# gio54321/quill-zkvm

Hardware: AMD Instinct MI355X
Metric: G1 MSM scalars/sec at 2^24 + sumcheck-prover ms at 2^20 vars (1/8 GPU) (higher is better)
Workload: dtype u256-montgomery (BN254 Fr scalars, Fq coordinates); 1 GPU; KZG commit / Pippenger G1 MSM, 2^24 BN254 scalars per GPU; parallelism=msm-shard-by-base-index x1

## Files before the change

quill-zkvm_amd/csrc/msm.hip:

```cpp
#include <stdlib.h>
#include <string.h>

#include "common.h"
#include "curve29.h"
#include "msm_plan.h"

using namespace qg;

namespace qg {

static constexpr int MSM_BLOCK = 256;

static int msm_window_bits(size_t n) {
  int best = 4;
  double best_cost = 1e300;
  for (int c = 4; c <= 22; c++) {
    const int W = (255 + c - 1) / c;
    const int k = 254 - c * (W - 1);
    if (k < 30 && (n >> k) > 4096) continue;
    const double cost = (double)n * W + 12.0 * (double)((size_t)1 << (c - 1));
    if (cost < best_cost) {
      best_cost = cost;
      best = c;
    }
// ... 86 lines not shown
    Fr s;
    if (canon_ready) {
      s = canon[i];
    } else {
      s = fr_canon29(scalars[i]);
      canon[i] = s;
    }
    for_each_digit(s, c, W, [&](int w, uint32_t b, bool) {
      if (wsel < 0 || w == wsel) atomicAdd(&hist[b >> LO], 1u);
    });
  }
  __syncthreads();
  for (int g = threadIdx.x; g < H; g += blockDim.x) hrow[(size_t)tb * H + g] = hist[g];
}

__global__ void __launch_bounds__(256)
    k_transpose32(const uint32_t* __restrict__ in, uint32_t rows, uint32_t cols,
                  uint32_t* __restrict__ out) {
  __shared__ uint32_t tile[32][33];
  const uint32_t c0 = blockIdx.x * 32, r0 = blockIdx.y * 32;
  const uint32_t tx = threadIdx.x & 31, ty = threadIdx.x >> 5;
  for (uint32_t k = ty; k < 32; k += 8)
    if (r0 + k < rows && c0 + tx < cols) tile[k][tx] = in[(size_t)(r0 + k) * cols + c0 + tx];
  __syncthreads();
  for (uint32_t k = ty; k < 32; k += 8)
    if (c0 + k < cols && r0 + tx < rows) out[(size_t)(c0 + k) * rows + r0 + tx] = tile[tx][k];
}

template <int BLK>
__device__ void lds_exscan(uint32_t* a, int n, uint32_t* tmp ) {
  const int per = (n + BLK - 1) / BLK;
  const int b = threadIdx.x * per;
  const int lane = threadIdx.x & 63, wid = threadIdx.x >> 6;
  uint32_t tot = 0;
  for (int k = 0; k < per; k++)
    if (b + k < n) tot += a[b + k];
  uint32_t inc = tot;
#pragma unroll
  for (int d = 1; d < 64; d <<= 1) {
    const uint32_t y = __shfl_up(inc, d, 64);
    if (lane >= d) inc += y;
// ... 149 lines not shown
      const uint32_t dst = gb[b >> LO] + p;
      tmp_e[dst] = ent[p];
      tmp_l[dst] = (uint16_t)(b & lmask);
    }
    if (!more) break;
    __syncthreads();
    k = kn;
    if (PF) {
#pragma unroll
      for (int j = 0; j < PER; j++) sv[j] = nsv[j];
      loff = nloff;
    }
  }
}

template <int BLK>
__global__ void __launch_bounds__(BLK)
    k_sortA_rows(uint32_t* __restrict__ hrow, uint32_t* __restrict__ orow, int H) {
  __shared__ uint32_t a[SORT_H_MAX], scr[BLK / 64];
  const size_t r = (size_t)blockIdx.x * H;
  for (int g = threadIdx.x; g < H; g += blockDim.x) a[g] = hrow[r + g];
  __syncthreads();
  lds_exscan<BLK>(a, H, scr);
  for (int g = threadIdx.x; g < H; g += blockDim.x) {
    hrow[r + g] = a[g];
    orow[r + g] -= a[g];
  }
}

__global__ void __launch_bounds__(1024)
    k_sort_chunks(const uint32_t* __restrict__ goff, uint32_t nblk, int H, uint32_t chunk,
                  uint32_t* __restrict__ gstart, uint32_t* __restrict__ cbase,
                  uint32_t* __restrict__ chunk_group, uint32_t* __restrict__ misc) {
  __shared__ uint32_t sh[1024];
  const int g = threadIdx.x;
  if (threadIdx.x >= 1 && threadIdx.x <= 3) misc[threadIdx.x] = threadIdx.x == 2 ? 0xffffffffu : 0u;
  const uint32_t total = goff[(size_t)H * nblk];
  uint32_t gs = 0, ge = 0, nch = 0;
  if (g < H) {
    gs = goff[(size_t)g * nblk];
    ge = (g + 1 < H) ? goff[(size_t)(g + 1) * nblk] : total;
    nch = (ge - gs + chunk - 1) / chunk;
    gstart[g] = gs;
  }
  sh[threadIdx.x] = nch;
  __syncthreads();
  for (int off = 1; off < 1024; off <<= 1) {
    uint32_t add = threadIdx.x >= (unsigned)off ? sh[threadIdx.x - off] : 0u;
    __syncthreads();
    sh[threadIdx.x] += add;
    __syncthreads();
  }
  const uint32_t cb = sh[threadIdx.x] - nch;
  if (g < H) {
    cbase[g] = cb;
    for (uint32_t k = 0; k < nch; k++) chunk_group[cb + k] = (uint32_t)g;
  }
  if (threadIdx.x == 1023) {
    gstart[H] = total;
    cbase[H] = sh[1023];
    misc[0] = sh[1023];
  }
}

template <int BLK, int CHUNK>
__global__ void __launch_bounds__(BLK)
    k_sortB_hist(const uint16_t* __restrict__ tmp_l, const uint32_t* __restrict__ gstart,
                 const uint32_t* __restrict__ cbase, const uint32_t* __restrict__ chunk_group,
                 const uint32_t* __restrict__ nchunks, int NL, uint32_t* __restrict__ chist) {
  extern __shared__ uint32_t hist[];
  const uint32_t nch = *nchunks;
  if (blockIdx.x >= nch) return;
  const uint32_t k = xcd_tile(blockIdx.x, nch);
  const uint32_t g = chunk_group[k];
  const uint32_t s = gstart[g] + (k - cbase[g]) * CHUNK;
  const uint32_t e = min(s + CHUNK, gstart[g + 1]);
// ... 15 lines not shown

__global__ void k_sort_bucket_count(const uint32_t* __restrict__ cbase, const uint32_t* __restrict__ chist,
                                    int LO, uint32_t nb, uint32_t* __restrict__ counts) {
  const uint32_t b = blockIdx.x * blockDim.x + threadIdx.x;
  if (b >= nb) return;
  const uint32_t g = b >> LO, l = b & ((1u << LO) - 1);
  uint32_t c = 0;
#pragma unroll 8
  for (uint32_t k = cbase[g]; k < cbase[g + 1]; k++) c += chist[((size_t)k << LO) + l];
  counts[b] = c;
}

__global__ void k_sort_chunk_offsets(const uint32_t* __restrict__ cbase,
                                     const uint32_t* __restrict__ chist, int LO, uint32_t nb,
                                     const uint32_t* __restrict__ bstart,
                                     uint32_t* __restrict__ coff) {
  const uint32_t b = blockIdx.x * blockDim.x + threadIdx.x;
  if (b >= nb) return;
  const uint32_t g = b >> LO, l = b & ((1u << LO) - 1);
  uint32_t run = bstart[b];
#pragma unroll 8
  for (uint32_t k = cbase[g]; k < cbase[g + 1]; k++) {
    const size_t idx = ((size_t)k << LO) + l;
    coff[idx] = run;
    run += chist[idx];
  }
}

template <int BLK, int CHUNK, bool PF>
__global__ void __launch_bounds__(BLK)
    k_sortB_scatter(const uint32_t* __restrict__ tmp_e, const uint16_t* __restrict__ tmp_l,
                    const uint32_t* __restrict__ gstart,
// ... 124 lines not shown
    if (PF) {
#pragma unroll
      for (int j = 0; j < PER; j++) {
        ev[j] = nev[j];
        lv[j] = nlv[j];
      }
#pragma unroll
      for (int r = 0; r < RPT; r++) co[r] = nco[r];
      loff = nloff;
      s = ns, e = ne;
      nck = fck, ns = fs, ne = fe;
    }
  }
}

__global__ void k_scan32_tiles(const uint32_t* __restrict__ in, size_t n, uint32_t* __restrict__ out,
                               uint32_t* __restrict__ tile_tot) {
  __shared__ uint32_t sh[256];
  const size_t base = ((size_t)blockIdx.x * 256 + threadIdx.x) * 8;
  uint32_t v[8], tot = 0;
  for (int k = 0; k < 8; k++) {
    v[k] = base + k < n ? in[base + k] : 0u;
    tot += v[k];
  }
  sh[threadIdx.x] = tot;
  __syncthreads();
  for (int off = 1; off < 256; off <<= 1) {
    uint32_t add = threadIdx.x >= (unsigned)off ? sh[threadIdx.x - off] : 0u;
    __syncthreads();
    sh[threadIdx.x] += add;
    __syncthreads();
  }
  uint32_t run = sh[threadIdx.x] - tot;
  for (int k = 0; k < 8; k++) {
    if (base + k < n) out[base + k] = run;
    run += v[k];
  }
  if (threadIdx.x == 255) tile_tot[blockIdx.x] = sh[255];
}

__global__ void __launch_bounds__(1024)
    k_scan32_top(uint32_t* __restrict__ tile_tot, int ntiles, uint32_t* __restrict__ out_total) {
  __shared__ uint32_t sh[1024];
  const int per = (ntiles + 1023) / 1024;
  const int base = threadIdx.x * per;
  uint32_t tot = 0;
  for (int k = 0; k < per; k++)
    if (base + k < ntiles) tot += tile_tot[base + k];
  sh[threadIdx.x] = tot;
  __syncthreads();
  for (int off = 1; off < 1024; off <<= 1) {
    uint32_t add = threadIdx.x >= (unsigned)off ? sh[threadIdx.x - off] : 0u;
    __syncthreads();
    sh[threadIdx.x] += add;
    __syncthreads();
  }
  uint32_t run = sh[threadIdx.x] - tot;
  for (int k = 0; k < per; k++) {
    if (base + k < ntiles) {
      uint32_t t = tile_tot[base + k];
      tile_tot[base + k] = run;
      run += t;
    }
  }
  if (threadIdx.x == 1023) *out_total = sh[1023];
}

__global__ void k_scan32_add(const uint32_t* __restrict__ tile_off, size_t n, uint32_t* __restrict__ out) {
  const size_t i = (size_t)blockIdx.x * blockDim.x + threadIdx.x;
  if (i < n) out[i] += tile_off[i / 2048];
}

__device__ __forceinline__ uint2 scan_val(const uint32_t* counts, size_t i, size_t nb, uint32_t L) {
  uint32_t c = i < nb ? counts[i] : 0u;
  return make_uint2(c, (c + L - 1) / L);
}

__global__ void k_scan_tiles(const uint32_t* __restrict__ counts, size_t nb, uint32_t L,
                             uint32_t* __restrict__ bstart, uint2* __restrict__ tile_tot,
                             uint32_t* __restrict__ max_tpb) {
  __shared__ uint2 sh[SCAN_BLOCK];
  size_t base = (size_t)blockIdx.x * SCAN_TILE + threadIdx.x * SCAN_PER_THREAD;
  uint2 v[SCAN_PER_THREAD];
  uint2 tot = make_uint2(0, 0);
  uint32_t mx = 0;
  for (int k = 0; k < SCAN_PER_THREAD; k++) {
    v[k] = scan_val(counts, base + k, nb, L);
    tot.x += v[k].x;
    tot.y += v[k].y;
    mx = max(mx, v[k].y);
  }
  if (mx > 1) atomicMax(max_tpb, mx);
  sh[threadIdx.x] = tot;
  __syncthreads();
  for (int off = 1; off < SCAN_BLOCK; off <<= 1) {
    uint2 add = threadIdx.x >= (unsigned)off ? sh[threadIdx.x - off] : make_uint2(0, 0);
    __syncthreads();
    sh[threadIdx.x].x += add.x;
    sh[threadIdx.x].y += add.y;
    __syncthreads();
  }
  uint2 run = threadIdx.x ? sh[threadIdx.x - 1] : make_uint2(0, 0);
  for (int k = 0; k < SCAN_PER_THREAD; k++) {
    size_t i = base + k;
    if (i < nb) bstart[i] = run.x;
    run.x += v[k].x;
    run.y += v[k].y;
// ... 453 lines not shown
    A_out[w] = x29_store(wsum);
    Y_out[w] = x29_store(Yw);
  }
#endif
}

QG_DEV G1Xyzz x29_export_xyzz(const X29& p) {
  if (x29_is_inf(p)) return G1Xyzz::infinity();
  return {q29_export(p.X), q29_export(p.Y), q29_export(p.ZZ), q29_export(p.ZZZ)};
}

template <bool Q4>
__global__ void __launch_bounds__(64)
    k_msm_wfold(const G1Xyzz* __restrict__ A_in, const G1Xyzz* __restrict__ Y_in, uint32_t m,
                size_t istride, G1Xyzz* __restrict__ A_out, G1Xyzz* __restrict__ Y_out,
                size_t ostride) {
#if defined(__HIP_DEVICE_COMPILE__)
  constexpr uint32_t ES = Q4 ? 4 : 1, G = 64 / ES;
  const uint32_t e0 = blockIdx.x * G, e = e0 + threadIdx.x / ES;
  const uint32_t mv = m - e0 < G ? m - e0 : G;
  X29 A = x29_inf(), Y = x29_inf();
  if (e < m) {
    A = x29_load(A_in[(size_t)blockIdx.y * istride + e]);
    Y = x29_load(Y_in[(size_t)blockIdx.y * istride + e]);
  }
  const int gl = Q4 ? 4 : 6;
  X29 Yw;
  msm_fold<Q4>(A, Y, gl, mv, 0, Y_out ? gl : 0, Yw);
  if (threadIdx.x == 0) {
    const size_t w = (size_t)blockIdx.y * ostride + blockIdx.x;
    if (Y_out) {
      A_out[w] = x29_store(A);
      Y_out[w] = x29_store(Yw);
    } else {
      A_out[w] = x29_export_xyzz(A);
    }
  }
#endif
}

__global__ void k_srs_pack(const G1Affine* __restrict__ pts, size_t n, MsmPt* __restrict__ out) {
  const size_t i = (size_t)blockIdx.x * blockDim.x + threadIdx.x;
  if (i >= n) return;
  const G1Affine w = pts[i];
  out[i] = w.is_inf() ? msm_pt_pack(Q29::zero(), Q29::zero(), true)
                      : msm_pt_pack(q29_import(w.x), q29_import(w.y), false);
}

__global__ void k_srs_unpack(const MsmPt* __restrict__ rows, size_t n, G1Affine* __restrict__ out) {
  const size_t i = (size_t)blockIdx.x * blockDim.x + threadIdx.x;
// ... 113 lines not shown
void srs_unpack_rows(qg_ctx* ctx, const qg_srs* srs, size_t offset, size_t n, G1Affine* d_out) {
  hipLaunchKernelGGL(k_srs_unpack, dim3(div_up(n, 256)), dim3(256), 0, ctx->stream,
                     srs->d_table + offset, n, d_out);
  QG_LAUNCH_CHECK();
}

struct MsmRun {
  bool empty = true;
  uint32_t L = 1, T = 4;
  size_t nslots = 0;
  X29Raw* partial = nullptr;
  uint32_t* owner = nullptr;
  uint32_t* bstart = nullptr;
  uint32_t* misc = nullptr;
  uint32_t* h_mx = nullptr;
  hipEvent_t ev_mx = nullptr;
  uint32_t gen = 0;
};
static constexpr int MSM_MAX_BATCH = 1024;

struct MsmJob {
  const Fr* d_scalars = nullptr;
  size_t n = 0;
  int slot = 0;
  size_t srs_off = 0;
  hipStream_t stream = nullptr;
  uint32_t* hv = nullptr;
  uint32_t hgen = 0;
  int wsel = -1;
  bool canon_ready = false;
// ... 24 lines not shown
  QG_HIP(hipFuncSetAttribute(f.fn, hipFuncAttributeMaxDynamicSharedMemorySize, 160 * 1024));
  ctx->memo[key] = "1";
}

static int sort_pf_occupancy(qg_ctx* ctx, char pass, int blk, size_t smem) {
  QG_CHECK(blk == 1024, QG_ERR_ASSERT, "the prefetching scatters have 1024 threads");
  const SortFn f = pass == 'A' ? sortA_fn<1024, true>() : sortB_fn<1024, 16384, true>();
  sort_lds_attr(ctx, f);
  const std::string mk = f.key + "_occ" + std::to_string(smem);
  auto it = ctx->memo.find(mk);
  if (it != ctx->memo.end()) return std::stoi(it->second);
  int occ = 0;
  QG_HIP(hipOccupancyMaxActiveBlocksPerMultiprocessor(&occ, f.fn, blk, smem));
  ctx->memo[mk] = std::to_string(occ);
  return occ;
}

static MsmPlan msm_job_plan(qg_ctx* ctx, const qg_srs* srs, const MsmJob& job) {
  const int W = srs->W, wsel = job.wsel;
  QG_CHECK((wsel < 0) == (srs->tables == W) && wsel < W, QG_ERR_INVALID,
           "MSM window selection does not match the SRS tables");
  QG_CHECK((size_t)W * srs->n < 0x80000000ull, QG_ERR_UNSUPPORTED, "SRS table index overflow");
  QG_CHECK(job.slot >= 0 && job.slot < MSM_MAX_BATCH, QG_ERR_UNSUPPORTED, "MSM batch too large");
  MsmShape sh;
  sh.n = job.n;
  sh.c = srs->c;
  sh.W = W;
  sh.wsel = wsel;
  sh.side = msm_on_side_stream(ctx, job);
  sh.cus = ctx->num_cus();
  return msm_plan(sh, msm_tuning_from_env(), [ctx](char pass, int blk, size_t smem) {
    return sort_pf_occupancy(ctx, pass, blk, smem);
  });
}

struct MsmScratch {
  uint32_t *ghist, *goff, *gtiles, *gstart, *cbase, *cgroup;
  uint32_t* misc;
  uint32_t *chist, *coff, *tmp_e;
  uint16_t* tmp_l;
  uint32_t *hrow, *orow;
  Fr* canon;
  uint32_t *counts, *bstart, *entries;
  uint2* tile_tot;
  X29Raw* partial;
  uint32_t* owner;
};

static MsmScratch msm_scratch(qg_ctx* ctx, const MsmPlan& p, size_t n, int slot, bool side,
                              bool run) {
  const std::string sfx = "#" + std::to_string(slot);
  const std::string tg = side ? "@" + std::to_string(slot & 1) : std::string();
  constexpr bool RESERVED = true, RUN_ONLY = false;
  auto get = [&](auto*& ptr, const std::string& name, size_t count, bool reserved) {
    using T = std::remove_reference_t<decltype(*ptr)>;
    if (run || reserved) ptr = ctx->scratch_as<T>(name, count);
  };
  MsmScratch s{};
  get(s.ghist, "msm_ghist" + tg, p.nghist + 1, RESERVED);
  get(s.goff, "msm_goff" + tg, p.nghist + 1, RESERVED);
  get(s.gtiles, "msm_gtiles" + tg, div_up(p.nghist, 2048) + 1, RESERVED);
  get(s.gstart, "msm_gstart" + tg, p.H + 1, RESERVED);
  get(s.cbase, "msm_cbase" + tg, p.H + 1, RESERVED);
  get(s.cgroup, "msm_cgroup" + tg, p.max_chunks, RESERVED);
  get(s.misc, "msm_misc" + sfx, 5, RESERVED);
  get(s.chist, "msm_chist" + tg, p.max_chunks * p.NL, RESERVED);
  get(s.coff, "msm_coff" + tg, p.max_chunks * p.NL, RESERVED);
  get(s.tmp_e, "msm_tmp_e" + tg, p.max_entries + 1, RESERVED);
  get(s.tmp_l, "msm_tmp_l" + tg, p.max_entries + 1, RESERVED);
  get(s.hrow, "msm_hrow" + tg, p.nghist + 1, RESERVED);
  get(s.orow, "msm_orow" + tg, p.nghist + 1, RESERVED);
  get(s.canon, "msm_canon" + tg, n, RESERVED);
  get(s.counts, "msm_counts" + tg, p.nb, RESERVED);
  get(s.bstart, "msm_bstart" + sfx, p.nb + 1, RESERVED);
  get(s.entries, "msm_entries" + tg, p.max_entries + 1, RESERVED);
  get(s.tile_tot, "msm_tiles" + tg, p.ntiles, RUN_ONLY);
  get(s.partial, "msm_partial" + sfx, p.nslots, RUN_ONLY);
  get(s.owner, "msm_owner" + sfx, p.nslots, RUN_ONLY);
  return s;
}
// ... 9 lines not shown
}

template <int BLK, bool PF>
static void launch_sortA_scatter(qg_ctx* ctx, const qg_srs* srs, const MsmJob& job,
                                 const MsmPlan& p, const MsmScratch& s) {
  sort_lds_attr(ctx, sortA_fn<BLK, PF>());
  hipLaunchKernelGGL(HIP_KERNEL_NAME(k_sortA_scatter<BLK, PF>), dim3(p.gridA), dim3(BLK), p.smemA,
                     job.stream, s.canon, job.n, srs->n, job.srs_off, srs->c, srs->W, p.LO, p.H,
                     p.nblk, p.geo.tile, s.hrow, s.orow, s.tmp_e, s.tmp_l, job.wsel,
                     PF ? 3u * (uint32_t)p.H : 0u);
  QG_LAUNCH_CHECK();
}
template <int BLK>
static void launch_sortA(qg_ctx* ctx, const qg_srs* srs, const MsmJob& job, const MsmPlan& p,
                         const MsmScratch& s) {
  hipLaunchKernelGGL(k_sortA_rows<BLK>, dim3(p.nblk), dim3(BLK), 0, job.stream, s.hrow, s.orow, p.H);
  QG_LAUNCH_CHECK();
  if (p.pfA)
    launch_sortA_scatter<1024, true>(ctx, srs, job, p, s);
  else
    launch_sortA_scatter<BLK, false>(ctx, srs, job, p, s);
}

template <int BLK, int CHUNK>
static void launch_sortB_hist(const MsmJob& job, const MsmPlan& p, const MsmScratch& s) {
  hipLaunchKernelGGL(HIP_KERNEL_NAME(k_sortB_hist<BLK, CHUNK>), dim3((unsigned)p.max_chunks),
                     dim3(BLK), p.NL * sizeof(uint32_t), job.stream, s.tmp_l, s.gstart, s.cbase,
                     s.cgroup, s.misc, p.NL, s.chist);
  QG_LAUNCH_CHECK();
}
template <int BLK, int CHUNK, bool PF>
static void launch_sortB_scatter_as(qg_ctx* ctx, const MsmJob& job, const MsmPlan& p,
// ... 29 lines not shown
  const bool small = p.geo.chunk == 8192;
  switch (p.geo.blkB) {
    case 256: launch_sortB_scatter<256, 8192>(ctx, job, p, s); break;
    case 512:
      if (small) launch_sortB_scatter<512, 8192>(ctx, job, p, s);
      else launch_sortB_scatter<512, 16384>(ctx, job, p, s);
      break;
    default: launch_sortB_scatter<1024, 16384>(ctx, job, p, s); break;
  }
}

static void msm_passA_launch(qg_ctx* ctx, const qg_srs* srs, const MsmJob& job, const MsmPlan& p,
                             const MsmScratch& s) {
  const hipStream_t st = job.stream;
  const uint32_t nblk = p.nblk, H = (uint32_t)p.H;
  hipLaunchKernelGGL(k_sortA_hist, dim3(nblk), dim3(SORT_BLOCK), H * sizeof(uint32_t), st,
                     job.d_scalars, job.n, srs->c, srs->W, p.LO, p.H, nblk, p.geo.tile, s.hrow,
                     s.canon, job.hv, job.hgen, job.wsel, job.canon_ready ? 1 : 0);
  QG_LAUNCH_CHECK();
  hipLaunchKernelGGL(k_transpose32, dim3(div_up(H, 32), div_up(nblk, 32)), dim3(256), 0, st, s.hrow,
                     nblk, H, s.ghist);
  QG_LAUNCH_CHECK();
  const unsigned gt = div_up(p.nghist, 2048);
  hipLaunchKernelGGL(k_scan32_tiles, dim3(gt), dim3(256), 0, st, s.ghist, p.nghist, s.goff, s.gtiles);
  QG_LAUNCH_CHECK();
  hipLaunchKernelGGL(k_scan32_top, dim3(1), dim3(1024), 0, st, s.gtiles, (int)gt, s.goff + p.nghist);
  QG_LAUNCH_CHECK();
  hipLaunchKernelGGL(k_scan32_add, dim3(div_up(p.nghist, 256)), dim3(256), 0, st, s.gtiles, p.nghist,
                     s.goff);
  QG_LAUNCH_CHECK();
  hipLaunchKernelGGL(k_transpose32, dim3(div_up(nblk, 32), div_up(H, 32)), dim3(256), 0, st, s.goff,
                     H, nblk, s.orow);
  QG_LAUNCH_CHECK();
  switch (p.geo.blkA) {
    case 256: launch_sortA<256>(ctx, srs, job, p, s); break;
    case 512: launch_sortA<512>(ctx, srs, job, p, s); break;
    default: launch_sortA<1024>(ctx, srs, job, p, s); break;
  }
}

static void msm_passB_launch(qg_ctx* ctx, const MsmJob& job, const MsmPlan& p, const MsmScratch& s,
                             const MsmRun& run) {
  const hipStream_t st = job.stream;
  const uint32_t nb = p.nb;
  hipLaunchKernelGGL(k_sort_chunks, dim3(1), dim3(1024), 0, st, s.goff, p.nblk, p.H, p.geo.chunk,
                     s.gstart, s.cbase, s.cgroup, s.misc);
  QG_LAUNCH_CHECK();
  sortB_hist_launch(job, p, s);
  hipLaunchKernelGGL(k_sort_bucket_count, dim3(div_up(nb, 256)), dim3(256), 0, st, s.cbase, s.chist,
                     p.LO, nb, s.counts);
  QG_LAUNCH_CHECK();
  hipLaunchKernelGGL(k_scan_tiles, dim3(p.ntiles), dim3(SCAN_BLOCK), 0, st, s.counts, (size_t)nb,
                     p.L, s.bstart, s.tile_tot, s.misc + 1);
  QG_LAUNCH_CHECK();
  hipLaunchKernelGGL(k_scan_top, dim3(1), dim3(1024), 0, st, s.tile_tot, p.ntiles, s.bstart,
                     (size_t)nb);
  QG_LAUNCH_CHECK();
  hipLaunchKernelGGL(k_scan_add, dim3(div_up(nb, 256)), dim3(256), 0, st, s.tile_tot, (size_t)nb,
                     s.bstart, s.counts, p.L, p.T, s.misc, run.gen, s.owner, p.nslots);
  QG_LAUNCH_CHECK();
  QG_HIP(hipMemcpyAsync(run.h_mx, s.misc + 1, 4 * sizeof(uint32_t), hipMemcpyDeviceToHost, st));
  QG_HIP(hipEventRecord(run.ev_mx, st));
  hipLaunchKernelGGL(k_sort_chunk_offsets, dim3(div_up(nb, 256)), dim3(256), 0, st, s.cbase, s.chist,
                     p.LO, nb, s.bstart, s.coff);
  QG_LAUNCH_CHECK();
  sortB_scatter_launch(ctx, job, p, s);
}

static void msm_bucketing_launch(qg_ctx* ctx, const qg_srs* srs, const MsmJob& job,
                                 const MsmPlan& p, const MsmScratch& s, const MsmRun& run) {
  QgTimed tm(ctx, msm_on_side_stream(ctx, job) ? "msm_bucketing_side" : "msm_bucketing", job.stream);
  msm_passA_launch(ctx, srs, job, p, s);
  msm_passB_launch(ctx, job, p, s, run);
}

static void msm_accumulate_launch(qg_ctx* ctx, const qg_srs* srs, const MsmJob& job,
                                  const MsmPlan& p, const MsmScratch& s) {
  QgTimed tm(ctx, "msm_accumulate", job.stream);
  auto kernel = p.coop ? k_msm_accumulate_coop : p.pf ? k_msm_accumulate<true> : k_msm_accumulate<false>;
  hipLaunchKernelGGL(kernel, dim3(div_up(p.max_threads, MSM_BLOCK)), dim3(MSM_BLOCK), 0, job.stream,
// ... 9 lines not shown
  MsmJob job = j;
  if (!job.stream) job.stream = ctx->stream;
  const MsmPlan p = msm_job_plan(ctx, srs, job);
  const MsmScratch s = msm_scratch(ctx, p, job.n, job.slot, msm_on_side_stream(ctx, job), true);
  uint32_t* hmx =
      reinterpret_cast<uint32_t*>(ctx->pinned_get("msm_mx", MSM_MAX_BATCH * 4 * sizeof(uint32_t)));
  run.empty = false;
  run.L = p.L;
  run.T = p.T;
  run.nslots = p.nslots;
  run.partial = s.partial;
  run.owner = s.owner;
  run.bstart = s.bstart;
  run.misc = s.misc;
  run.h_mx = hmx + 4 * job.slot;
  run.ev_mx = evs.get();
  run.gen = ++ctx->msm_gen;
  msm_bucketing_launch(ctx, srs, job, p, s, run);
  msm_accumulate_launch(ctx, srs, job, p, s);
  return run;
}

struct MsmHandover {
  uint32_t* hv = nullptr;
  uint32_t hgen = 0;
  uint32_t* h_err = nullptr;
};

static void msm_reduce_phase(qg_ctx* ctx, const qg_srs* srs, const std::vector<MsmRun>& runs,
                             std::vector<G1Xyzz>& out, const MsmHandover& ho = {}) {
// ... 36 lines not shown
  const size_t lanes = (size_t)ctx->num_cus() * 4 * 64;
  int slog1 = 0;
  while (slog1 < 12 && ((size_t)kl * nb >> (slog1 + 1)) >= lanes) slog1++;
  if (const char* ov = getenv("QG_MSM_SLOG1")) slog1 = atoi(ov);
  QG_CHECK(slog1 >= 0 && slog1 <= 12, QG_ERR_INVALID, "QG_MSM_SLOG1 out of range");
  int gl1 = 4;
  if (const char* ov = getenv("QG_MSM_GL1")) gl1 = atoi(ov);
  QG_CHECK(gl1 >= 0 && gl1 <= 6, QG_ERR_INVALID, "QG_MSM_GL1 out of range");
  const uint32_t g1 = div_up(div_up(nb, (size_t)1 << slog1), MSM_BLOCK);
  const uint32_t m1 = g1 * (MSM_BLOCK >> gl1);
  const uint32_t m2 = div_up(m1, 16);
  G1Xyzz* A1 = ctx->scratch_as<G1Xyzz>("msm_redA1", (size_t)kl * m1);
  G1Xyzz* Y1 = ctx->scratch_as<G1Xyzz>("msm_redY1", (size_t)kl * m1);
  G1Xyzz* A2 = ctx->scratch_as<G1Xyzz>("msm_redA2", (size_t)kl * m2);
  G1Xyzz* Y2 = ctx->scratch_as<G1Xyzz>("msm_redY2", (size_t)kl * m2);
  G1Xyzz* d_out = ctx->scratch_as<G1Xyzz>("msm_out", kl);
  std::vector<MsmRed> h_runs(kl);
  MsmRedSet rset{};
  {
    QgTimed tm(ctx, "msm_reduce");
    for (uint32_t q = 0; q < kl; q++) {
      const MsmRun& r = runs[live[q]];
      const uint32_t max_slots = mx[3 * q] + 1, s_lo = mx[3 * q + 1], s_hi = mx[3 * q + 2];
      uint32_t st = 1;
      while (s_lo <= s_hi && (size_t)st * r.T < max_slots) {
        QG_CHECK(s_hi < r.nslots, QG_ERR_ASSERT, "MSM partial-slot range");
        hipLaunchKernelGGL(k_msm_tree_step, dim3(div_up(s_hi - s_lo + 1, MSM_BLOCK)), dim3(MSM_BLOCK),
                           0, ctx->stream, r.partial, r.owner, r.bstart, r.L, r.T, s_lo, s_hi + 1,
                           st, hv, hgen);
        QG_LAUNCH_CHECK();
        st <<= 1;
// ... 10 lines not shown
      d_runs = d;
    }
    hipLaunchKernelGGL(k_msm_bsum, dim3(g1, kl), dim3(MSM_BLOCK), 0, ctx->stream, d_runs, rset, nb,
                       slog1, gl1, A1, Y1, (size_t)m1, hv, hgen);
    QG_LAUNCH_CHECK();
    G1Xyzz *Ai = A1, *Yi = Y1, *Ao = A2, *Yo = Y2;
    size_t istride = m1;
    uint32_t m = m1;
    bool q4 = true;
    if (const char* ov = getenv("QG_MSM_Q4")) q4 = atoi(ov) != 0;
    const uint32_t per = q4 ? 16 : 64;
    auto fold = q4 ? k_msm_wfold<true> : k_msm_wfold<false>;
    while (m > per) {
      const uint32_t mo = div_up(m, per);
      hipLaunchKernelGGL(fold, dim3(mo, kl), dim3(64), 0, ctx->stream, Ai, Yi, m, istride, Ao, Yo,
                         (size_t)mo);
      QG_LAUNCH_CHECK();
      std::swap(Ai, Ao);
      std::swap(Yi, Yo);
      istride = mo;
      m = mo;
    }
    hipLaunchKernelGGL(fold, dim3(1, kl), dim3(64), 0, ctx->stream, Ai, Yi, m, istride, d_out,
                       (G1Xyzz*)nullptr, (size_t)1);
    QG_LAUNCH_CHECK();
  }
  std::vector<G1Xyzz> h(kl);
  QG_HIP(hipMemcpyAsync(h.data(), d_out, kl * sizeof(G1Xyzz), hipMemcpyDeviceToHost, ctx->stream));
  if (hv) QG_HIP(hipMemcpyAsync(h_err, hv + 1, sizeof(uint32_t), hipMemcpyDeviceToHost, ctx->stream));
  ctx->sync();
  for (uint32_t q = 0; q < kl; q++) out[live[q]] = h[q];
}

static G1Affine msm_finish_ranks(qg_ctx* ctx, G1Xyzz acc) {
  if (ctx->sharded) {
    G1Xyzz* d_send = ctx->scratch_as<G1Xyzz>("msm_comm_send", 1);
    G1Xyzz* d_recv = ctx->scratch_as<G1Xyzz>("msm_comm_recv", ctx->world);
    QG_HIP(hipMemcpyAsync(d_send, &acc, sizeof(G1Xyzz), hipMemcpyHostToDevice, ctx->stream));
    comm_allgather_bytes(ctx, d_send, d_recv, sizeof(G1Xyzz));
    std::vector<G1Xyzz> all(ctx->world);
    QG_HIP(hipMemcpyAsync(all.data(), d_recv, sizeof(G1Xyzz) * ctx->world, hipMemcpyDeviceToHost,
                          ctx->stream));
    ctx->sync();
    acc = G1Xyzz::infinity();
    for (int r = 0; r < ctx->world; r++) acc = xyzz_add(acc, all[r]);
  }
// ... 273 lines not shown
                         uint32_t* Y_out) {
  if (!ctx || !A || !Y || !A_out || (want_y && !Y_out)) return QG_ERR_INVALID;
  if (m == 0 || m > X29_MAX_CASES || batch == 0 || batch > 16) return QG_ERR_INVALID;
  if (istride < m || istride > X29_MAX_CASES) return QG_ERR_INVALID;
  return qg_guard(ctx, [&] {
    static_assert(sizeof(G1Xyzz) == 32 * sizeof(uint32_t), "XYZZ word layout");
    QG_HIP(hipSetDevice(ctx->device));
    const uint32_t per = q4 ? 16 : 64, mo = div_up(m, per);
    const size_t ni = (size_t)batch * istride, no = (size_t)batch * mo;
    G1Xyzz* d = ctx->scratch_as<G1Xyzz>("fold_selftest", 2 * ni + 2 * no);
    G1Xyzz *dA = d, *dY = d + ni, *dAo = d + 2 * ni, *dYo = dAo + no;
    QG_HIP(hipMemcpyAsync(dA, A, ni * sizeof(G1Xyzz), hipMemcpyHostToDevice, ctx->stream));
    QG_HIP(hipMemcpyAsync(dY, Y, ni * sizeof(G1Xyzz), hipMemcpyHostToDevice, ctx->stream));
    auto fold = q4 ? k_msm_wfold<true> : k_msm_wfold<false>;
    hipLaunchKernelGGL(fold, dim3(mo, batch), dim3(64), 0, ctx->stream, dA, dY, m, istride, dAo,
                       want_y ? dYo : (G1Xyzz*)nullptr, (size_t)mo);
    QG_LAUNCH_CHECK();
    QG_HIP(hipMemcpyAsync(A_out, dAo, no * sizeof(G1Xyzz), hipMemcpyDeviceToHost, ctx->stream));
    if (want_y)
      QG_HIP(hipMemcpyAsync(Y_out, dYo, no * sizeof(G1Xyzz), hipMemcpyDeviceToHost, ctx->stream));
    ctx->sync();
  });
}

int qg_microbench_fetch(qg_ctx* ctx, size_t rows, size_t gathers, double* gather_ms,
                        double* stream_ms) {
  if (!ctx || !rows || !gathers || !gather_ms || !stream_ms || rows > 0xffffffffull)
    return QG_ERR_INVALID;
  return qg_guard(ctx, [&] {
    QG_HIP(hipSetDevice(ctx->device));
    MsmPt* table = ctx->scratch_as<MsmPt>("mb_fetch_table", rows);
// ... 260 lines not shown
```

Measured before the change: 941.4 million scalars/s.

## Fuse pass-A histogram offset scan into strip kernels and drop small copies

Replaces the transpose, three-kernel scan, transpose-back and the per-row exscan and chunk-planning kernels of sort pass A with a strip-sum kernel, a hierarchical top scan that uses a last-block counter to also build chunk metadata, and a strip-local row scan. Device-to-host memcpys for the max-tiles counters, the final MSM result and the error flag are replaced by kernel writes into mapped pinned memory. A wave-level max reduction also cuts global atomics in the scan. The aim is to remove many small dispatches, launch gaps and copy-engine operations from the MSM critical path. In exchange it adds cross-block counter synchronisation that must be re-armed per slot, and system-scope writes to host memory.

```diff
diff --git a/profiles/msm_chain_spans.py b/profiles/msm_chain_spans.py
--- /dev/null
+++ b/profiles/msm_chain_spans.py
@@ -0,0 +1,88 @@
+import csv
+import re
+import sys
+
+LARGE = ("k_sortA_hist", "k_sortA_scatter", "k_sortB_hist", "k_sortB_scatter",
+         "k_msm_accumulate", "k_msm_bsum")
+MSM_KERNELS = re.compile(r"k_sort|k_scan|k_transpose32|k_msm_(accumulate|tree_step|bsum|wfold|fold)"
+                         r"|__amd_rocclr_copyBuffer|k_handover_tag")
+
+
+def short(name):
+    m = re.search(r"(?:qg::)?(k_\w+|__amd_rocclr_\w+)", name)
+    return m.group(1) if m else name
+
+
+def is_large(k):
+    return any(k.startswith(x) for x in LARGE)
+
+
+def chain_of(k, seen):
+    if "k_sortA_scatter" not in seen:
+        return "passA"
+    if "k_sortB_scatter" not in seen:
+        return "bscan"
+    return "tail"
+
+
+def main():
+    rows = []
+    with open(sys.argv[1]) as f:
+        for r in csv.DictReader(f):
+            k = short(r["Kernel_Name"])
+            if not MSM_KERNELS.search(k):
+                continue
+            rows.append((int(r["Start_Timestamp"]), int(r["End_Timestamp"]), k,
+                         (int(r["Grid_Size_X"]), int(r["Grid_Size_Y"])), int(r["Workgroup_Size_X"])))
+    rows.sort()
+    msms, cur = [], None
+    for r in rows:
+        if r[2] == "k_sortA_hist":
+            cur = []
+            msms.append(cur)
+        if cur is not None:
+            cur.append(r)
+    label = sys.argv[2] if len(sys.argv) > 2 else ""
+    last_by_grid = {}
+    for m in msms:
+        acc = [r for r in m if r[2].startswith("k_msm_accumulate")]
+        if acc:
+            last_by_grid[acc[0][3]] = m
+    for m in last_by_grid.values():
+        end = max(i for i, r in enumerate(m) if r[2].startswith(("k_msm_wfold", "k_msm_fold", "k_msm_bsum")))
+        while end + 1 < len(m) and m[end + 1][2].startswith("__amd_rocclr") and \
+                m[end + 1][0] - m[end][1] < 100000:
+            end += 1
+        m = m[:end + 1]
+        t0 = m[0][0]
+        total = m[-1][1] - t0
+        print(f"== {label} lone MSM, accumulate grid {m[[r[2].startswith('k_msm_accumulate') for r in m].index(True)][3][0]}:"
+              f" {len(m)} dispatches, first start to last end {total / 1e3:.1f} us")
+        print(f"{'start_us':>10} {'end_us':>10} {'dur_us':>8} {'gap_us':>7}  grid wg  kernel  [chain]")
+        seen, prev_end = set(), None
+        span = {"passA": [0, 0, 0], "bscan": [0, 0, 0], "tail": [0, 0, 0]}
+        large = 0
+        for s, e, k, g, wg in m:
+            gap = 0 if prev_end is None else s - prev_end
+            big = is_large(k)
+            ch = chain_of(k, seen)
+            if big:
+                large += e - s
+                if prev_end is not None:
+                    span[ch][1] += gap
+            else:
+                span[ch][0] += e - s
+                span[ch][1] += gap
+                span[ch][2] += 1
+            print(f"{(s - t0) / 1e3:10.1f} {(e - t0) / 1e3:10.1f} {(e - s) / 1e3:8.1f} {gap / 1e3:7.1f}  "
+                  f"{g[0]}x{g[1]} {wg}  {k}  [{'large' if big else ch}]")
+            seen.add(k.split("<")[0])
+            prev_end = e
+        print(f"six large kernels: {large / 1e3:.1f} us; span outside them: {(total - large) / 1e3:.1f} us")
+        for ch, (kt, gp, nd) in span.items():
+            print(f"  {ch:6s}: {nd:2d} small dispatches, kernels {kt / 1e3:7.1f} us + gaps {gp / 1e3:6.1f} us"
+                  f" = {(kt + gp) / 1e3:7.1f} us")
+
+
+if __name__ == "__main__":
+    main()
diff --git a/quill-zkvm_amd/csrc/msm.hip b/quill-zkvm_amd/csrc/msm.hip
--- a/quill-zkvm_amd/csrc/msm.hip
+++ b/quill-zkvm_amd/csrc/msm.hip
@@ -124,17 +124,23 @@
   for (int g = threadIdx.x; g < H; g += blockDim.x) hrow[(size_t)tb * H + g] = hist[g];
 }
 
-__global__ void __launch_bounds__(256)
-    k_transpose32(const uint32_t* __restrict__ in, uint32_t rows, uint32_t cols,
-                  uint32_t* __restrict__ out) {
-  __shared__ uint32_t tile[32][33];
-  const uint32_t c0 = blockIdx.x * 32, r0 = blockIdx.y * 32;
-  const uint32_t tx = threadIdx.x & 31, ty = threadIdx.x >> 5;
-  for (uint32_t k = ty; k < 32; k += 8)
-    if (r0 + k < rows && c0 + tx < cols) tile[k][tx] = in[(size_t)(r0 + k) * cols + c0 + tx];
+__device__ __forceinline__ bool msm_last_block(uint32_t* counter, uint32_t nblocks, uint32_t* flag) {
+  asm volatile("s_waitcnt vmcnt(0)" ::: "memory");
   __syncthreads();
-  for (uint32_t k = ty; k < 32; k += 8)
-    if (c0 + k < cols && r0 + tx < rows) out[(size_t)(c0 + k) * rows + r0 + tx] = tile[tx][k];
+  if (threadIdx.x == 0) {
+    __builtin_amdgcn_fence(__ATOMIC_RELEASE, "agent");
+    asm volatile("s_waitcnt vmcnt(0)" ::: "memory");
+    const uint32_t t = __hip_atomic_fetch_add(counter, 1u, __ATOMIC_RELAXED, __HIP_MEMORY_SCOPE_AGENT);
+    const bool last = t + 1 == nblocks;
+    if (last) {
+      __hip_atomic_store(counter, 0u, __ATOMIC_RELAXED, __HIP_MEMORY_SCOPE_AGENT);
+      __builtin_amdgcn_fence(__ATOMIC_ACQUIRE, "agent");
+      asm volatile("s_waitcnt vmcnt(0)" ::: "memory");
+    }
+    *flag = last ? 1u : 0u;
+  }
+  __syncthreads();
+  return *flag != 0u;
 }
 
 template <int BLK>
@@ -314,52 +320,162 @@
   }
 }
 
+static constexpr int SORTA_STRIP_WORDS = 8192;
+static constexpr uint32_t SORTA_SUP = 32, SORTA_STRIPS_MIN = 512, SORTA_SIDE_ROWS = 4;
+static uint32_t sortA_strip_rows(int H, uint32_t nblk, bool side) {
+  const uint32_t rmax = std::min<uint32_t>(32u, (uint32_t)(SORTA_STRIP_WORDS / H));
+  uint32_t r = std::max<uint32_t>(1u, std::min<uint32_t>(rmax, nblk / SORTA_STRIPS_MIN));
+  if (side) r = std::min(r, SORTA_SIDE_ROWS);
+  if (const char* ov = getenv("QG_SORT_STRIP_ROWS")) {
+    const int v = atoi(ov);
+    QG_CHECK(v >= 1 && (uint32_t)v <= rmax, QG_ERR_INVALID, "QG_SORT_STRIP_ROWS out of range");
+    r = (uint32_t)v;
+  }
+  return r;
+}
+
+__global__ void __launch_bounds__(256)
+    k_sortA_strips(const uint32_t* __restrict__ hrow, uint32_t nblk, int H, uint32_t R,
+                   uint32_t* __restrict__ ssum) {
+  const uint32_t s = blockIdx.x, t0 = s * R;
+  const uint32_t rows = nblk - t0 < R ? nblk - t0 : R;
+  for (int g = threadIdx.x; g < H; g += blockDim.x) {
+    uint32_t sum = 0;
+#pragma unroll 8
+    for (uint32_t r = 0; r < rows; r++) sum += hrow[(size_t)(t0 + r) * H + g];
+    ssum[(size_t)s * H + g] = sum;
+  }
+}
+
 template <int BLK>
 __global__ void __launch_bounds__(BLK)
-    k_sortA_rows(uint32_t* __restrict__ hrow, uint32_t* __restrict__ orow, int H) {
-  __shared__ uint32_t a[SORT_H_MAX], scr[BLK / 64];
-  const size_t r = (size_t)blockIdx.x * H;
-  for (int g = threadIdx.x; g < H; g += blockDim.x) a[g] = hrow[r + g];
+    k_sortA_top(uint32_t* ssum, uint32_t* usum, uint32_t nstrips, int H, uint32_t chunk,
+                uint32_t* counter, uint32_t* __restrict__ gstart, uint32_t* __restrict__ cbase,
+                uint32_t* __restrict__ chunk_group, uint32_t* __restrict__ misc) {
+  constexpr int PER = SORT_H_MAX / BLK, NWAVE = BLK / 64;
+  __shared__ uint32_t wtot[NWAVE];
+  __shared__ uint32_t last;
+  const uint32_t u = blockIdx.x, s0 = u * SORTA_SUP;
+  const uint32_t s1 = nstrips - s0 < SORTA_SUP ? nstrips : s0 + SORTA_SUP;
+  for (int g = threadIdx.x; g < H; g += blockDim.x) {
+    uint32_t v[SORTA_SUP];
+#pragma unroll
+    for (uint32_t k = 0; k < SORTA_SUP; k++) v[k] = s0 + k < s1 ? ssum[(size_t)(s0 + k) * H + g] : 0u;
+    uint32_t run = 0;
+#pragma unroll
+    for (uint32_t k = 0; k < SORTA_SUP; k++) {
+      if (s0 + k < s1) ssum[(size_t)(s0 + k) * H + g] = run;
+      run += v[k];
+    }
+    usum[(size_t)u * H + g] = run;
+  }
+  if (!msm_last_block(counter, gridDim.x, &last)) return;
+  if (threadIdx.x >= 1 && threadIdx.x <= 3) misc[threadIdx.x] = threadIdx.x == 2 ? 0xffffffffu : 0u;
+  const int g0 = (int)threadIdx.x * PER;
+  uint32_t tot[PER];
+#pragma unroll
+  for (int j = 0; j < PER; j++) {
+    tot[j] = 0;
+    const int g = g0 + j;
+    if (g >= H) continue;
+    for (uint32_t v0 = 0; v0 < gridDim.x; v0 += 16) {
+      uint32_t x[16];
+#pragma unroll
+      for (uint32_t k = 0; k < 16; k++) x[k] = v0 + k < gridDim.x ? usum[(size_t)(v0 + k) * H + g] : 0u;
+#pragma unroll
+      for (uint32_t k = 0; k < 16; k++) {
+        if (v0 + k < gridDim.x) usum[(size_t)(v0 + k) * H + g] = tot[j];
+        tot[j] += x[k];
+      }
+    }
+  }
+  const uint32_t lane = threadIdx.x & 63u, wid = threadIdx.x >> 6;
+  auto block_scan = [&](uint32_t x, uint32_t& all) {
+    uint32_t inc = x;
+#pragma unroll
+    for (int d = 1; d < 64; d <<= 1) {
+      const uint32_t y = __shfl_up(inc, d, 64);
+      if (lane >= (uint32_t)d) inc += y;
+    }
+    __syncthreads();
+    if (lane == 63) wtot[wid] = inc;
+    __syncthreads();
+    all = 0;
+    for (uint32_t w = 0; w < NWAVE; w++) {
+      if (w < wid) inc += wtot[w];
+      all += wtot[w];
+    }
+    return inc;
+  };
+  uint32_t tsum = 0, nch[PER], csum = 0;
+#pragma unroll
+  for (int j = 0; j < PER; j++) {
+    tsum += tot[j];
+    nch[j] = (tot[j] + chunk - 1) / chunk;
+    csum += nch[j];
+  }
+  uint32_t total, nchunks;
+  uint32_t gs = block_scan(tsum, total) - tsum;
+  uint32_t cb = block_scan(csum, nchunks) - csum;
+#pragma unroll
+  for (int j = 0; j < PER; j++) {
+    const int g = g0 + j;
+    if (g < H) {
+      gstart[g] = gs;
+      cbase[g] = cb;
+      for (uint32_t k = 0; k < nch[j]; k++) chunk_group[cb + k] = (uint32_t)g;
+    }
+    gs += tot[j];
+    cb += nch[j];
+  }
+  if (threadIdx.x == 0) {
+    gstart[H] = total;
+    cbase[H] = nchunks;
+    misc[0] = nchunks;
+  }
+}
+
+__global__ void __launch_bounds__(512)
+    k_sortA_rows(uint32_t* __restrict__ hrow, uint32_t* __restrict__ orow,
+                 const uint32_t* __restrict__ ssum, const uint32_t* __restrict__ usum,
+                 const uint32_t* __restrict__ gstart, uint32_t nblk, int H_, uint32_t R) {
+  const uint32_t H = (uint32_t)H_;
+  extern __shared__ uint32_t strip[];
+  uint32_t* const a = strip;
+  uint32_t* const cb = strip + R * H;
+  const uint32_t s = blockIdx.x, t0 = s * R;
+  const uint32_t rows = nblk - t0 < R ? nblk - t0 : R;
+  const size_t r0 = (size_t)t0 * H;
+  const uint32_t nw = rows * H;
+  for (uint32_t i = threadIdx.x; i < nw; i += blockDim.x) a[i] = hrow[r0 + i];
   __syncthreads();
-  lds_exscan<BLK>(a, H, scr);
-  for (int g = threadIdx.x; g < H; g += blockDim.x) {
-    hrow[r + g] = a[g];
-    orow[r + g] -= a[g];
-  }
-}
-
-__global__ void __launch_bounds__(1024)
-    k_sort_chunks(const uint32_t* __restrict__ goff, uint32_t nblk, int H, uint32_t chunk,
-                  uint32_t* __restrict__ gstart, uint32_t* __restrict__ cbase,
-                  uint32_t* __restrict__ chunk_group, uint32_t* __restrict__ misc) {
-  __shared__ uint32_t sh[1024];
-  const int g = threadIdx.x;
-  if (threadIdx.x >= 1 && threadIdx.x <= 3) misc[threadIdx.x] = threadIdx.x == 2 ? 0xffffffffu : 0u;
-  const uint32_t total = goff[(size_t)H * nblk];
-  uint32_t gs = 0, ge = 0, nch = 0;
-  if (g < H) {
-    gs = goff[(size_t)g * nblk];
-    ge = (g + 1 < H) ? goff[(size_t)(g + 1) * nblk] : total;
-    nch = (ge - gs + chunk - 1) / chunk;
-    gstart[g] = gs;
-  }
-  sh[threadIdx.x] = nch;
+  for (uint32_t g = threadIdx.x; g < H; g += blockDim.x) {
+    uint32_t run = gstart[g] + usum[(size_t)(s / SORTA_SUP) * H + g] + ssum[(size_t)s * H + g];
+    for (uint32_t r = 0; r < rows; r++) {
+      cb[r * H + g] = run;
+      run += a[r * H + g];
+    }
+  }
   __syncthreads();
-  for (int off = 1; off < 1024; off <<= 1) {
-    uint32_t add = threadIdx.x >= (unsigned)off ? sh[threadIdx.x - off] : 0u;
-    __syncthreads();
-    sh[threadIdx.x] += add;
-    __syncthreads();
-  }
-  const uint32_t cb = sh[threadIdx.x] - nch;
-  if (g < H) {
-    cbase[g] = cb;
-    for (uint32_t k = 0; k < nch; k++) chunk_group[cb + k] = (uint32_t)g;
-  }
-  if (threadIdx.x == 1023) {
-    gstart[H] = total;
-    cbase[H] = sh[1023];
-    misc[0] = sh[1023];
+  const uint32_t lane = threadIdx.x & 63u, wid = threadIdx.x >> 6, nwav = blockDim.x >> 6;
+  for (uint32_t r = wid; r < rows; r += nwav) {
+    uint32_t carry = 0;
+    for (uint32_t k0 = 0; k0 < H; k0 += 64) {
+      const uint32_t g = k0 + lane;
+      const uint32_t v = g < H ? a[r * H + g] : 0u;
+      uint32_t inc = v;
+#pragma unroll
+      for (int d = 1; d < 64; d <<= 1) {
+        const uint32_t y = __shfl_up(inc, d, 64);
+        if (lane >= (uint32_t)d) inc += y;
+      }
+      const uint32_t ex = carry + inc - v;
+      if (g < H) {
+        hrow[r0 + r * H + g] = ex;
+        orow[r0 + r * H + g] = cb[r * H + g] - ex;
+      }
+      carry += __shfl(inc, 63, 64);
+    }
   }
 }
 
@@ -405,8 +521,13 @@
 __global__ void k_sort_chunk_offsets(const uint32_t* __restrict__ cbase,
                                      const uint32_t* __restrict__ chist, int LO, uint32_t nb,
                                      const uint32_t* __restrict__ bstart,
-                                     uint32_t* __restrict__ coff) {
+                                     uint32_t* __restrict__ coff, const uint32_t* __restrict__ misc,
+                                     uint32_t* __restrict__ h_mx) {
   const uint32_t b = blockIdx.x * blockDim.x + threadIdx.x;
+  if (b == 0) {
+    for (int i = 0; i < 3; i++) h_mx[i] = misc[1 + i];
+    __hip_atomic_store(h_mx + 3, misc[4], __ATOMIC_RELEASE, __HIP_MEMORY_SCOPE_SYSTEM);
+  }
   if (b >= nb) return;
   const uint32_t g = b >> LO, l = b & ((1u << LO) - 1);
   uint32_t run = bstart[b];
@@ -561,63 +682,6 @@
   }
 }
 
-__global__ void k_scan32_tiles(const uint32_t* __restrict__ in, size_t n, uint32_t* __restrict__ out,
-                               uint32_t* __restrict__ tile_tot) {
-  __shared__ uint32_t sh[256];
-  const size_t base = ((size_t)blockIdx.x * 256 + threadIdx.x) * 8;
-  uint32_t v[8], tot = 0;
-  for (int k = 0; k < 8; k++) {
-    v[k] = base + k < n ? in[base + k] : 0u;
-    tot += v[k];
-  }
-  sh[threadIdx.x] = tot;
-  __syncthreads();
-  for (int off = 1; off < 256; off <<= 1) {
-    uint32_t add = threadIdx.x >= (unsigned)off ? sh[threadIdx.x - off] : 0u;
-    __syncthreads();
-    sh[threadIdx.x] += add;
-    __syncthreads();
-  }
-  uint32_t run = sh[threadIdx.x] - tot;
-  for (int k = 0; k < 8; k++) {
-    if (base + k < n) out[base + k] = run;
-    run += v[k];
-  }
-  if (threadIdx.x == 255) tile_tot[blockIdx.x] = sh[255];
-}
-
-__global__ void __launch_bounds__(1024)
-    k_scan32_top(uint32_t* __restrict__ tile_tot, int ntiles, uint32_t* __restrict__ out_total) {
-  __shared__ uint32_t sh[1024];
-  const int per = (ntiles + 1023) / 1024;
-  const int base = threadIdx.x * per;
-  uint32_t tot = 0;
-  for (int k = 0; k < per; k++)
-    if (base + k < ntiles) tot += tile_tot[base + k];
-  sh[threadIdx.x] = tot;
-  __syncthreads();
-  for (int off = 1; off < 1024; off <<= 1) {
-    uint32_t add = threadIdx.x >= (unsigned)off ? sh[threadIdx.x - off] : 0u;
-    __syncthreads();
-    sh[threadIdx.x] += add;
-    __syncthreads();
-  }
-  uint32_t run = sh[threadIdx.x] - tot;
-  for (int k = 0; k < per; k++) {
-    if (base + k < ntiles) {
-      uint32_t t = tile_tot[base + k];
-      tile_tot[base + k] = run;
-      run += t;
-    }
-  }
-  if (threadIdx.x == 1023) *out_total = sh[1023];
-}
-
-__global__ void k_scan32_add(const uint32_t* __restrict__ tile_off, size_t n, uint32_t* __restrict__ out) {
-  const size_t i = (size_t)blockIdx.x * blockDim.x + threadIdx.x;
-  if (i < n) out[i] += tile_off[i / 2048];
-}
-
 __device__ __forceinline__ uint2 scan_val(const uint32_t* counts, size_t i, size_t nb, uint32_t L) {
   uint32_t c = i < nb ? counts[i] : 0u;
   return make_uint2(c, (c + L - 1) / L);
@@ -637,7 +701,9 @@
     tot.y += v[k].y;
     mx = max(mx, v[k].y);
   }
-  if (mx > 1) atomicMax(max_tpb, mx);
+#pragma unroll
+  for (int d = 32; d >= 1; d >>= 1) mx = max(mx, (uint32_t)__shfl_xor(mx, d, 64));
+  if ((threadIdx.x & 63) == 0 && mx > 1) atomicMax(max_tpb, mx);
   sh[threadIdx.x] = tot;
   __syncthreads();
   for (int off = 1; off < SCAN_BLOCK; off <<= 1) {
@@ -1121,7 +1187,7 @@
 __global__ void __launch_bounds__(64)
     k_msm_wfold(const G1Xyzz* __restrict__ A_in, const G1Xyzz* __restrict__ Y_in, uint32_t m,
                 size_t istride, G1Xyzz* __restrict__ A_out, G1Xyzz* __restrict__ Y_out,
-                size_t ostride) {
+                size_t ostride, const uint32_t* hv, uint32_t* __restrict__ h_err) {
 #if defined(__HIP_DEVICE_COMPILE__)
   constexpr uint32_t ES = Q4 ? 4 : 1, G = 64 / ES;
   const uint32_t e0 = blockIdx.x * G, e = e0 + threadIdx.x / ES;
@@ -1141,6 +1207,8 @@
       Y_out[w] = x29_store(Yw);
     } else {
       A_out[w] = x29_export_xyzz(A);
+      if (h_err && w == 0)
+        *h_err = __hip_atomic_load(hv + 1, __ATOMIC_RELAXED, __HIP_MEMORY_SCOPE_AGENT);
     }
   }
 #endif
@@ -1284,6 +1352,7 @@
   uint32_t* bstart = nullptr;
   uint32_t* misc = nullptr;
   uint32_t* h_mx = nullptr;
+  uint32_t* d_mx = nullptr;
   hipEvent_t ev_mx = nullptr;
   uint32_t gen = 0;
 };
@@ -1338,6 +1407,22 @@
   QG_HIP(hipOccupancyMaxActiveBlocksPerMultiprocessor(&occ, f.fn, blk, smem));
   ctx->memo[mk] = std::to_string(occ);
   return occ;
+}
+
+template <class T>
+static T* pinned_dev(T* host) {
+  void* d = nullptr;
+  QG_HIP(hipHostGetDevicePointer(&d, host, 0));
+  return reinterpret_cast<T*>(d);
+}
+
+static void msm_counters_arm(qg_ctx* ctx, int slot, uint32_t* ctr, hipStream_t st) {
+  const std::string name = "msm_ctr#" + std::to_string(slot);
+  const std::string gen = std::to_string(ctx->scratch_gen(name));
+  auto it = ctx->memo.find(name);
+  if (it != ctx->memo.end() && it->second == gen) return;
+  QG_HIP(hipMemsetAsync(ctr, 0, 4 * sizeof(uint32_t), st));
+  ctx->memo[name] = gen;
 }
 
 static MsmPlan msm_job_plan(qg_ctx* ctx, const qg_srs* srs, const MsmJob& job) {
@@ -1359,8 +1444,9 @@
 }
 
 struct MsmScratch {
-  uint32_t *ghist, *goff, *gtiles, *gstart, *cbase, *cgroup;
+  uint32_t *ssum, *usum, *gstart, *cbase, *cgroup;
   uint32_t* misc;
+  uint32_t* ctr;
   uint32_t *chist, *coff, *tmp_e;
   uint16_t* tmp_l;
   uint32_t *hrow, *orow;
@@ -1381,13 +1467,13 @@
     if (run || reserved) ptr = ctx->scratch_as<T>(name, count);
   };
   MsmScratch s{};
-  get(s.ghist, "msm_ghist" + tg, p.nghist + 1, RESERVED);
-  get(s.goff, "msm_goff" + tg, p.nghist + 1, RESERVED);
-  get(s.gtiles, "msm_gtiles" + tg, div_up(p.nghist, 2048) + 1, RESERVED);
+  get(s.ssum, "msm_ssum" + tg, p.nghist + SORT_H_MAX, RESERVED);
+  get(s.usum, "msm_usum" + tg, div_up(p.nghist, SORTA_SUP) + SORT_H_MAX, RESERVED);
   get(s.gstart, "msm_gstart" + tg, p.H + 1, RESERVED);
   get(s.cbase, "msm_cbase" + tg, p.H + 1, RESERVED);
   get(s.cgroup, "msm_cgroup" + tg, p.max_chunks, RESERVED);
   get(s.misc, "msm_misc" + sfx, 5, RESERVED);
+  get(s.ctr, "msm_ctr" + sfx, 4, RUN_ONLY);
   get(s.chist, "msm_chist" + tg, p.max_chunks * p.NL, RESERVED);
   get(s.coff, "msm_coff" + tg, p.max_chunks * p.NL, RESERVED);
   get(s.tmp_e, "msm_tmp_e" + tg, p.max_entries + 1, RESERVED);
@@ -1427,8 +1513,6 @@
 template <int BLK>
 static void launch_sortA(qg_ctx* ctx, const qg_srs* srs, const MsmJob& job, const MsmPlan& p,
                          const MsmScratch& s) {
-  hipLaunchKernelGGL(k_sortA_rows<BLK>, dim3(p.nblk), dim3(BLK), 0, job.stream, s.hrow, s.orow, p.H);
-  QG_LAUNCH_CHECK();
   if (p.pfA)
     launch_sortA_scatter<1024, true>(ctx, srs, job, p, s);
   else
@@ -1488,23 +1572,21 @@
                              const MsmScratch& s) {
   const hipStream_t st = job.stream;
   const uint32_t nblk = p.nblk, H = (uint32_t)p.H;
+  const bool side = msm_on_side_stream(ctx, job);
+  const uint32_t R = sortA_strip_rows(p.H, nblk, side), nstrips = div_up(nblk, R);
   hipLaunchKernelGGL(k_sortA_hist, dim3(nblk), dim3(SORT_BLOCK), H * sizeof(uint32_t), st,
                      job.d_scalars, job.n, srs->c, srs->W, p.LO, p.H, nblk, p.geo.tile, s.hrow,
                      s.canon, job.hv, job.hgen, job.wsel, job.canon_ready ? 1 : 0);
   QG_LAUNCH_CHECK();
-  hipLaunchKernelGGL(k_transpose32, dim3(div_up(H, 32), div_up(nblk, 32)), dim3(256), 0, st, s.hrow,
-                     nblk, H, s.ghist);
+  hipLaunchKernelGGL(k_sortA_strips, dim3(nstrips), dim3(256), 0, st, s.hrow, nblk, p.H, R, s.ssum);
   QG_LAUNCH_CHECK();
-  const unsigned gt = div_up(p.nghist, 2048);
-  hipLaunchKernelGGL(k_scan32_tiles, dim3(gt), dim3(256), 0, st, s.ghist, p.nghist, s.goff, s.gtiles);
+  hipLaunchKernelGGL(side ? k_sortA_top<256> : k_sortA_top<1024>, dim3(div_up(nstrips, SORTA_SUP)),
+                     dim3(side ? 256 : 1024), 0, st, s.ssum, s.usum, nstrips, p.H, p.geo.chunk, s.ctr,
+                     s.gstart, s.cbase, s.cgroup, s.misc);
   QG_LAUNCH_CHECK();
-  hipLaunchKernelGGL(k_scan32_top, dim3(1), dim3(1024), 0, st, s.gtiles, (int)gt, s.goff + p.nghist);
-  QG_LAUNCH_CHECK();
-  hipLaunchKernelGGL(k_scan32_add, dim3(div_up(p.nghist, 256)), dim3(256), 0, st, s.gtiles, p.nghist,
-                     s.goff);
-  QG_LAUNCH_CHECK();
-  hipLaunchKernelGGL(k_transpose32, dim3(div_up(nblk, 32), div_up(H, 32)), dim3(256), 0, st, s.goff,
-                     H, nblk, s.orow);
+  hipLaunchKernelGGL(k_sortA_rows, dim3(nstrips), dim3(R > SORTA_SIDE_ROWS ? 512 : 256),
+                     2 * R * H * sizeof(uint32_t), st, s.hrow, s.orow, s.ssum, s.usum, s.gstart, nblk,
+                     p.H, R);
   QG_LAUNCH_CHECK();
   switch (p.geo.blkA) {
     case 256: launch_sortA<256>(ctx, srs, job, p, s); break;
@@ -1517,9 +1599,6 @@
                              const MsmRun& run) {
   const hipStream_t st = job.stream;
   const uint32_t nb = p.nb;
-  hipLaunchKernelGGL(k_sort_chunks, dim3(1), dim3(1024), 0, st, s.goff, p.nblk, p.H, p.geo.chunk,
-                     s.gstart, s.cbase, s.cgroup, s.misc);
-  QG_LAUNCH_CHECK();
   sortB_hist_launch(job, p, s);
   hipLaunchKernelGGL(k_sort_bucket_count, dim3(div_up(nb, 256)), dim3(256), 0, st, s.cbase, s.chist,
                      p.LO, nb, s.counts);
@@ -1533,11 +1612,10 @@
   hipLaunchKernelGGL(k_scan_add, dim3(div_up(nb, 256)), dim3(256), 0, st, s.tile_tot, (size_t)nb,
                      s.bstart, s.counts, p.L, p.T, s.misc, run.gen, s.owner, p.nslots);
   QG_LAUNCH_CHECK();
-  QG_HIP(hipMemcpyAsync(run.h_mx, s.misc + 1, 4 * sizeof(uint32_t), hipMemcpyDeviceToHost, st));
+  hipLaunchKernelGGL(k_sort_chunk_offsets, dim3(div_up(nb, 256)), dim3(256), 0, st, s.cbase, s.chist,
+                     p.LO, nb, s.bstart, s.coff, s.misc, run.d_mx);
+  QG_LAUNCH_CHECK();
   QG_HIP(hipEventRecord(run.ev_mx, st));
-  hipLaunchKernelGGL(k_sort_chunk_offsets, dim3(div_up(nb, 256)), dim3(256), 0, st, s.cbase, s.chist,
-                     p.LO, nb, s.bstart, s.coff);
-  QG_LAUNCH_CHECK();
   sortB_scatter_launch(ctx, job, p, s);
 }
 
@@ -1577,6 +1655,8 @@
   run.bstart = s.bstart;
   run.misc = s.misc;
   run.h_mx = hmx + 4 * job.slot;
+  run.d_mx = pinned_dev(hmx) + 4 * job.slot;
+  msm_counters_arm(ctx, job.slot, s.ctr, job.stream);
   run.ev_mx = evs.get();
   run.gen = ++ctx->msm_gen;
   msm_bucketing_launch(ctx, srs, job, p, s, run);
@@ -1643,7 +1723,9 @@
   G1Xyzz* Y1 = ctx->scratch_as<G1Xyzz>("msm_redY1", (size_t)kl * m1);
   G1Xyzz* A2 = ctx->scratch_as<G1Xyzz>("msm_redA2", (size_t)kl * m2);
   G1Xyzz* Y2 = ctx->scratch_as<G1Xyzz>("msm_redY2", (size_t)kl * m2);
-  G1Xyzz* d_out = ctx->scratch_as<G1Xyzz>("msm_out", kl);
+  G1Xyzz* h_out =
+      reinterpret_cast<G1Xyzz*>(ctx->pinned_get("msm_out_h", MSM_MAX_BATCH * sizeof(G1Xyzz)));
+  G1Xyzz* d_out = pinned_dev(h_out);
   std::vector<MsmRed> h_runs(kl);
   MsmRedSet rset{};
   {
@@ -1684,7 +1766,7 @@
     while (m > per) {
       const uint32_t mo = div_up(m, per);
       hipLaunchKernelGGL(fold, dim3(mo, kl), dim3(64), 0, ctx->stream, Ai, Yi, m, istride, Ao, Yo,
-                         (size_t)mo);
+                         (size_t)mo, (const uint32_t*)nullptr, (uint32_t*)nullptr);
       QG_LAUNCH_CHECK();
       std::swap(Ai, Ao);
       std::swap(Yi, Yo);
@@ -1692,14 +1774,12 @@
       m = mo;
     }
     hipLaunchKernelGGL(fold, dim3(1, kl), dim3(64), 0, ctx->stream, Ai, Yi, m, istride, d_out,
-                       (G1Xyzz*)nullptr, (size_t)1);
+                       (G1Xyzz*)nullptr, (size_t)1, (const uint32_t*)hv,
+                       hv ? pinned_dev(h_err) : (uint32_t*)nullptr);
     QG_LAUNCH_CHECK();
   }
-  std::vector<G1Xyzz> h(kl);
-  QG_HIP(hipMemcpyAsync(h.data(), d_out, kl * sizeof(G1Xyzz), hipMemcpyDeviceToHost, ctx->stream));
-  if (hv) QG_HIP(hipMemcpyAsync(h_err, hv + 1, sizeof(uint32_t), hipMemcpyDeviceToHost, ctx->stream));
   ctx->sync();
-  for (uint32_t q = 0; q < kl; q++) out[live[q]] = h[q];
+  for (uint32_t q = 0; q < kl; q++) out[live[q]] = h_out[q];
 }
 
 static G1Affine msm_finish_ranks(qg_ctx* ctx, G1Xyzz acc) {
@@ -2003,7 +2083,8 @@
     QG_HIP(hipMemcpyAsync(dY, Y, ni * sizeof(G1Xyzz), hipMemcpyHostToDevice, ctx->stream));
     auto fold = q4 ? k_msm_wfold<true> : k_msm_wfold<false>;
     hipLaunchKernelGGL(fold, dim3(mo, batch), dim3(64), 0, ctx->stream, dA, dY, m, istride, dAo,
-                       want_y ? dYo : (G1Xyzz*)nullptr, (size_t)mo);
+                       want_y ? dYo : (G1Xyzz*)nullptr, (size_t)mo, (const uint32_t*)nullptr,
+                       (uint32_t*)nullptr);
     QG_LAUNCH_CHECK();
     QG_HIP(hipMemcpyAsync(A_out, dAo, no * sizeof(G1Xyzz), hipMemcpyDeviceToHost, ctx->stream));
     if (want_y)
```

After: 948.8 million scalars/s, median of 6. About the same (+0.8%).
